# telegraphroad/VCNF

Hardware: AMD Instinct MI355X
Metric: flow transforms/sec (log_prob + sample), D=64 RQ-spline, batch=1M (higher is better)
Workload: dtype f32 results on fp16x3 split operands: every fp32 operand of a conditioner GEMM travels as hi + lo fp16 halves, three f16 matrix instructions per product (four in the 48- and 16-deep layers), fp32 accumulation; measured against fp64 (tests/test_gpu_gemm_error.py): GEMM error 0.6-0.75x the exact-fp32

## Files before the change

### vcnf_amd/csrc/fused_layer_v6.hip

```cpp
#include <hip/hip_runtime.h>
#include <stdint.h>

#include "../../include/vcnf_hip.h"
#include "rqs_math.hpp"
#include "fused_common.hpp"
#include "host_common.hpp"
#include "rqs_lean.hpp"
#include "split_half.hpp"

#ifndef VCNF_ABL
#define VCNF_ABL 0
#endif
#ifndef VCNF_TIME
#define VCNF_TIME 0
#endif
#ifndef VCNF_AHEAD
#define VCNF_AHEAD 1
#endif
#if VCNF_TIME
#define VCNF_T(I) { const long long t_ = clock64(); tacc[I] += t_ - tlast; tlast = t_; }
#define VCNF_TIME_PARAM , float* tstamps
#define VCNF_TIME_ARG , time_buffer()
#else
#define VCNF_T(I)
#define VCNF_TIME_PARAM
#define VCNF_TIME_ARG
#endif

#define VCNF_SYNC() { __builtin_amdgcn_sched_barrier(0); asm volatile("s_waitcnt lgkmcnt(0)\n\ts_barrier" ::: "memory"); __builtin_amdgcn_sched_barrier(0); }

namespace vcnf {

#if VCNF_TIME
constexpr int kTimeSlots = 24;
static float* time_buffer() {
  static float* buf = nullptr;
  if (!buf && hipMalloc(&buf, 2 * kTimeSlots * sizeof(float)) != hipSuccess) buf = nullptr;
  return buf;
}
extern "C" int vcnf_v6_phase_stamps(float* out) {
  if (!time_buffer() || hipDeviceSynchronize() != hipSuccess) return VCNF_ERR_LAUNCH;
  return hipMemcpy(out, time_buffer(), 2 * kTimeSlots * sizeof(float), hipMemcpyDeviceToHost) == hipSuccess ? VCNF_OK : VCNF_ERR_LAUNCH;
}
#endif

template <int DI, int DT, int C, int H, int NBLK, int K, bool INV>
__global__ __launch_bounds__(512, 2) void fused_rqs_layer_v6_kernel(const FusedArgs a VCNF_TIME_PARAM) {
  static_assert(H == 128 && K == 8, "4 row blocks of 32 over 4 waves; 3 K - 1 = 23 logits: two features per 48 rows");
  static_assert((DI == 16 || DI == 32) && DT == DI && (C == 0 || C == 16), "shape family");
  constexpr int kBlock = 512;
  constexpr int kTile = 128;
  constexpr int NCB = 4;
  constexpr int D = DI + DT;
  constexpr int XS = D + 4;
  constexpr int NTX = DI / 16;
  constexpr int NTC = C / 16;
  constexpr int NT0 = NTX + NTC;
  constexpr int NTH = H / 16;
  constexpr int P = 3 * K - 1;
  constexpr int NG = DT / 4;
  constexpr int NR = NG / 2;
  constexpr int TABW = 3 * (K + 1);
  using L = PackLayout6<DI, DT, C, H, NBLK, K>;
  constexpr int GFRAG = 3 * NTH * 2 * 64;
  constexpr int RING = VCNF_AHEAD + 1;

  extern __shared__ __align__(16) float smem[];
  using S = LdsV6<DI, DT, C, H, NBLK, K>;
  static_assert(S::TILE == kTile && S::FRAG_N == 2 * GFRAG * 4 && S::XT_N == kTile * XS && S::TAB_N >= DI * TABW, "layout");
  uint4* act = reinterpret_cast<uint4*>(smem + S::FRAG);
  uint4* act_hi = act;
  uint4* act_lo = act + NTH * NCB * 64;
  float* xt = smem + S::XT;
  uint4* ctxf = reinterpret_cast<uint4*>(smem + S::CTXF);
  float* tab = smem + S::TAB;
  float* ldt = smem + S::LDT;
  int* tfi = reinterpret_cast<int*>(smem + S::TFI);
  int* idi = reinterpret_cast<int*>(smem + S::IDI);
  constexpr int NBV = C > 0 ? 3 : 2;
  constexpr int NBT = S::NBT;
  constexpr int BPL = S::BPL;
  float* biasf = smem + S::BIAS;
  float* ldold = smem + S::LDOLD;
  int* tflag = reinterpret_cast<int*>(smem + S::TFLAG);

  const int tid = threadIdx.x;
  const int lane = tid & 63;
  const int wave = __builtin_amdgcn_readfirstlane(tid >> 6);
  const int rp = wave & 3;
  const int ch = wave >> 2;
  const int c32 = lane & 31;
  const int kg = lane >> 5;
  const RqsConst& c = a.c;
  const bool shared = a.sh_w != nullptr;
  const LeanConst lc = make_lean_const(c);

  if (ch == 1) __builtin_amdgcn_s_setprio(1);
  for (int i = tid; i < NG * 96; i += kBlock) {
    const int g = i / 96, hf = i % 96 / 48;
    biasf[hf * BPL + g * 48 + i % 48] = a.wpack[L::BF + i];
  }
  for (int i = tid; i < NBT * H; i += kBlock) {
    const int v = i / H, blk = (v - 1) / NBV, sel = (v - 1) % NBV, r = i % H;
    const int off = v == 0 ? L::B0 : L::BLK0 + blk * L::BLK + (sel == 0 ? L::BA : sel == 1 ? L::BB : L::BC);
    biasf[(r >> 4 & 1) * BPL + NG * 48 + v * (H / 2) + (r >> 5) * 16 + (r & 15)] = a.wpack[off + r];
  }
  for (int i = tid; i < DT; i += kBlock) tfi[i] = a.tf_idx[i];
  for (int i = tid; i < DI; i += kBlock) idi[i] = a.id_idx[i];
  if (shared) {
    for (int i = tid; i < 3 * DI; i += kBlock) {
      const int f = i % DI;
      SplitLogits p{a.sh_w + f * K, a.sh_h + f * K, a.sh_d + f * (K - 1), K, 1.f, c.edge_logit, c.tails};
      rqs_build_table_part_k<K>(p, c, tab + f * TABW, 1, i / DI);
    }
  }

  const __amdgpu_buffer_rsrc_t wr =
      __builtin_amdgcn_make_buffer_rsrc(const_cast<float*>(a.wpack), 0, a.wpack_bytes, 0x00020000);
  const int voff = lane * 16;
  const float* bplane = biasf + kg * BPL;

  const long long ntiles = (a.B + kTile - 1) / kTile;
  bool bad = false;
  float satm = 0.f;
#if VCNF_TIME
  long long tacc[20], tlast = clock64();
  const long long tstart = tlast, rstart = wall_clock64();
  for (int i = 0; i < 20; ++i) tacc[i] = 0;
#endif
  float4 xpre[kTile * (D / 4) / kBlock], cpre[1];
  static_assert(kTile * (D / 4) % kBlock == 0 && (C == 0 || kTile * (C / 4) == kBlock), "rows per thread");
#define VCNF_PREFETCH_ROWS(TILE)                                                          \
  {                                                                                       \
    const long long pb0 = min((TILE) * kTile, a.B);                                       \
    const long long left = (a.B - pb0) * (D * 4);                                         \
    const __amdgpu_buffer_rsrc_t xr_ = __builtin_amdgcn_make_buffer_rsrc(                 \
        const_cast<float*>(a.x) + pb0 * D, 0, (int)min(left, (long long)(kTile * D * 4)), 0x00020000); \
    _Pragma("unroll") for (int k = 0; k < kTile * (D / 4) / kBlock; ++k)                  \
      xpre[k] = __builtin_bit_cast(float4, __builtin_amdgcn_raw_buffer_load_b128(xr_, (tid + kBlock * k) * 16, 0, 0)); \
    if (C > 0) {                                                                          \
      const long long leftc = (a.B - pb0) * (C * 4);                                      \
      const __amdgpu_buffer_rsrc_t cr_ = __builtin_amdgcn_make_buffer_rsrc(               \
          const_cast<float*>(a.ctx) + pb0 * C, 0, (int)min(leftc, (long long)(kTile * C * 4)), 0x00020000); \
      cpre[0] = __builtin_bit_cast(float4, __builtin_amdgcn_raw_buffer_load_b128(cr_, tid * 16, 0, 0)); \
    }                                                                                     \
  }
#define VCNF_ROWS_ARRIVED()                                                               \
  {                                                                                       \
    _Pragma("unroll") for (int k = 0; k < kTile * (D / 4) / kBlock; ++k) {                \
      floatx4 v_ = __builtin_bit_cast(floatx4, xpre[k]);                                  \
      asm volatile("" : "+v"(v_));                                                        \
      xpre[k] = __builtin_bit_cast(float4, v_);                                           \
    }                                                                                     \
    if (C > 0) {                                                                          \
      floatx4 v_ = __builtin_bit_cast(floatx4, cpre[0]);                                  \
      asm volatile("" : "+v"(v_));                                                        \
      cpre[0] = __builtin_bit_cast(float4, v_);                                           \
    }                                                                                     \
  }
  VCNF_PREFETCH_ROWS((long long)blockIdx.x)
  VCNF_ROWS_ARRIVED()
  for (long long tile = blockIdx.x; tile < ntiles; tile += gridDim.x) {
    const long long b0 = tile * kTile;
    const int rows = (int)min((long long)kTile, a.B - b0);
    satm = 0.f;
    { VCNF_T(0) VCNF_SYNC(); VCNF_T(15) }
    {
      constexpr int D4 = D / 4;
      if (tid == 0) *tflag = 0;
#pragma unroll
      for (int k = 0; k < kTile * D4 / kBlock; ++k) {
        const int i = tid + kBlock * k;
        const int r = i / D4, o = i - r * D4;
        *reinterpret_cast<float4*>(xt + r * XS + 4 * o) = xpre[k];
      }
      if (C > 0) {
        const int r = tid >> 2, part = tid & 3;
        half4 h4, l4;
        const float cv[4] = {cpre[0].x, cpre[0].y, cpre[0].z, cpre[0].w};
#pragma unroll
        for (int i = 0; i < 4; ++i) satm = fmaxf(satm, cv[i] == cv[i] ? __builtin_fabsf(cv[i]) : __builtin_inff());
        asm volatile("" : "+v"(satm));
#pragma unroll
        for (int i = 0; i < 4; ++i) {
          const float x = __builtin_amdgcn_fmed3f(cv[i], -65504.f, 65504.f);
          const _Float16 hv = (_Float16)x;
          h4[i] = hv;
          l4[i] = (_Float16)((x - (float)hv) * kLoScale);
        }
        const int at = (((r >> 5) * 2) * 64 + (r & 31) + 32 * (part >> 1));
        uint2* dh = reinterpret_cast<uint2*>(ctxf + at) + (part & 1);
        uint2* dl = reinterpret_cast<uint2*>(ctxf + at + 64) + (part & 1);
        *dh = __builtin_bit_cast(uint2, h4);
        *dl = __builtin_bit_cast(uint2, l4);
      }
    }
    { VCNF_T(1) VCNF_SYNC(); VCNF_T(15) }

    {
      constexpr int UNR = DI / 4;
      const int mi = tid >> 2, part = tid & 3;
      float lsum = 0.f;
      float xv[UNR], fv[UNR];
      float* px[UNR];
#pragma unroll
      for (int k = 0; k < UNR; ++k) {
        px[k] = xt + mi * XS + idi[part * UNR + k];
        xv[k] = *px[k];
        fv[k] = xv[k];
      }
      if (shared) {
        float yv[UNR], lad[UNR];
        bool in_[UNR];
#pragma unroll
        for (int k = 0; k < UNR; ++k) {
          in_[k] = (xv[k] >= c.lo_x) && (xv[k] <= c.hi_x);
          bool bad1 = false;
          rqs_point_table_inside<INV, K>(in_[k] ? xv[k] : c.lo_x, tab + (part * UNR + k) * TABW, yv[k], lad[k], bad1);
          bad = bad || (bad1 && in_[k]);
        }
#pragma unroll
        for (int k = 0; k < UNR; ++k) {
          const float o = in_[k] ? yv[k] : xv[k];
          *px[k] = o;
          if (INV) fv[k] = o;
          lsum += in_[k] ? lad[k] : 0.f;
        }
      }
      lsum += __shfl_xor(lsum, 1, 64);
      lsum += __shfl_xor(lsum, 2, 64);
      int tid_ = tid;
      asm volatile("" : "+v"(tid_));
      if (part == 0) ldt[tid_ >> 2] = lsum;
#pragma unroll
      for (int k = 0; k < UNR; ++k) satm = fmaxf(satm, fv[k] == fv[k] ? 0.f : __builtin_inff());
      const int k0 = part * UNR;
      const int t0 = k0 >> 4, kg0 = (k0 >> 3) & 1;
      const int at = (t0 * NCB + (mi >> 5)) * 64 + (mi & 31) + 32 * kg0;
      if (UNR == 8) {
        half8 h8, l8;
        float f8[8];
#pragma unroll
        for (int k = 0; k < 8; ++k) f8[k] = fv[k < UNR ? k : 0];
        split8<false>(f8, h8, l8, satm);
        act_hi[at] = __builtin_bit_cast(uint4, h8);
        act_lo[at] = __builtin_bit_cast(uint4, l8);
      } else {
        half4 h4, l4;
        satm = fmaxf(fmaxf(satm, __builtin_fabsf(fv[0])), __builtin_fabsf(fv[1]));
        satm = fmaxf(fmaxf(satm, __builtin_fabsf(fv[2 < UNR ? 2 : 0])), __builtin_fabsf(fv[3 < UNR ? 3 : 0]));
        asm volatile("" : "+v"(satm));
#pragma unroll
        for (int i = 0; i < 4; ++i) {
          const float x = __builtin_amdgcn_fmed3f(fv[i < UNR ? i : 0], -65504.f, 65504.f);
          const _Float16 hv = (_Float16)x;
          h4[i] = hv;
          l4[i] = (_Float16)((x - (float)hv) * kLoScale);
        }
        reinterpret_cast<uint2*>(act_hi + at)[(k0 >> 2) & 1] = __builtin_bit_cast(uint2, h4);
        reinterpret_cast<uint2*>(act_lo + at)[(k0 >> 2) & 1] = __builtin_bit_cast(uint2, l4);
      }
    }
    { VCNF_T(2) VCNF_SYNC(); VCNF_T(15) }
    if (ch == 1) { VCNF_T(14) VCNF_SYNC(); VCNF_T(16) }

    half8 ahi[NTH], alo[NTH];
    floatx16 abias;
#define VCNF_LOAD_BIAS16(DST, VEC)                                                        \
  _Pragma("unroll") for (int i_ = 0; i_ < 4; ++i_) {                                      \
    const floatx4 b4_ = *reinterpret_cast<const floatx4*>(bplane + NG * 48 + (VEC) * (H / 2) + 16 * rp + 4 * i_); \
    DST[4 * i_ + 0] = b4_[0]; DST[4 * i_ + 1] = b4_[1]; DST[4 * i_ + 2] = b4_[2]; DST[4 * i_ + 3] = b4_[3]; \
  }
#define VCNF_LOAD_HIDDEN(WOFF, BVEC)                                                      \
  {                                                                                       \
    _Pragma("unroll") for (int t = 0; t < NTH; ++t) {                                     \
      ahi[t] = __builtin_bit_cast(half8, wload(wr, voff, 4 * ((WOFF) + ((rp * NTH + t) * 2 + 0) * 256))); \
      alo[t] = __builtin_bit_cast(half8, wload(wr, voff, 4 * ((WOFF) + ((rp * NTH + t) * 2 + 1) * 256))); \
    }                                                                                     \
    VCNF_LOAD_BIAS16(abias, BVEC)                                                         \
  }

    floatx16 h[2];
    {
      half8 w0h[NT0], w0l[NT0];
      floatx16 bias0;
#pragma unroll
      for (int t = 0; t < NT0; ++t) {
        w0h[t] = __builtin_bit_cast(half8, wload(wr, voff, 4 * (L::W0 + ((rp * NT0 + t) * 2 + 0) * 256)));
        w0l[t] = __builtin_bit_cast(half8, wload(wr, voff, 4 * (L::W0 + ((rp * NT0 + t) * 2 + 1) * 256)));
      }
      VCNF_LOAD_BIAS16(bias0, 0)
#pragma unroll
      for (int j = 0; j < 2; ++j) {
        const int cb = 2 * ch + j;
        floatx16 mainv = bias0, corr = {}, corr2 = {};
#pragma unroll
        for (int t = 0; t < NT0; ++t) {
          const half8 bh = __builtin_bit_cast(half8, t < NTX ? act_hi[(t * NCB + cb) * 64 + lane] : ctxf[(cb * 2 + 0) * 64 + lane]);
          const half8 bl = __builtin_bit_cast(half8, t < NTX ? act_lo[(t * NCB + cb) * 64 + lane] : ctxf[(cb * 2 + 1) * 64 + lane]);
          mainv = mfma32h(w0h[t], bh, mainv);
          corr = mfma32h(w0h[t], bl, corr);
          corr = mfma32h(w0l[t], bh, corr);
          corr2 = mfma32h(w0l[t], bl, corr2);
        }
#pragma unroll
        for (int r = 0; r < 16; ++r) h[j][r] = fmaf(fmaf(corr2[r], kLoUnscale, corr[r]), kLoUnscale, mainv[r]);
      }
    }
    { VCNF_T(3) VCNF_SYNC(); VCNF_T(15) }
#define VCNF_PUBLISH(SRC, RELU)                                                           \
  _Pragma("unroll") for (int j = 0; j < 2; ++j) {                                         \
    _Pragma("unroll") for (int hh = 0; hh < 2; ++hh) {                                    \
      float v8_[8];                                                                       \
      _Pragma("unroll") for (int i = 0; i < 8; ++i) v8_[i] = SRC[j][8 * hh + i];          \
      half8 h8_, l8_;                                                                     \
      split8<RELU>(v8_, h8_, l8_, satm);                                                  \
      const int at = ((2 * rp + hh) * NCB + 2 * ch + j) * 64 + lane;                      \
      act_hi[at] = __builtin_bit_cast(uint4, h8_);                                        \
      act_lo[at] = __builtin_bit_cast(uint4, l8_);                                        \
    }                                                                                     \
  }
    VCNF_LOAD_HIDDEN(L::BLK0 + L::WA, 1)
    VCNF_PUBLISH(h, true)
    { VCNF_T(4) VCNF_SYNC(); VCNF_T(15) }

#define VCNF_READ_B(T)                                                                    \
  {                                                                                       \
    rh[(T) % RING] = __builtin_bit_cast(half8, act_hi[((((T) & 7)) * NCB + 2 * ch + ((T) >> 3)) * 64 + lane]); \
    rl[(T) % RING] = __builtin_bit_cast(half8, act_lo[((((T) & 7)) * NCB + 2 * ch + ((T) >> 3)) * 64 + lane]); \
  }
#define VCNF_HIDDEN_COMPUTE(OUT)                                                          \
  {                                                                                       \
    half8 rh[RING], rl[RING];                 \
    floatx16 corr;                                                                        \
    _Pragma("unroll") for (int st_ = 0; st_ < VCNF_AHEAD; ++st_) {                        \
      VCNF_READ_B(st_)                                                                    \
    }                                                                                     \
    _Pragma("unroll") for (int st_ = 0; st_ < 2 * NTH; ++st_) {                           \
      const int j = st_ >> 3, tk_ = st_ & 7;                                              \
      if (st_ + VCNF_AHEAD < 2 * NTH) {                                                   \
        VCNF_READ_B(st_ + VCNF_AHEAD)                                                     \
      }                                                                                   \
      if (tk_ == 0) {                                                                       \
        OUT[j] = abias;                                                                   \
        corr = floatx16{};                                                                \
      }                                                                                   \
      OUT[j] = mfma32h(ahi[tk_], rh[st_ % RING], OUT[j]);                                      \
      corr = mfma32h(ahi[tk_], rl[st_ % RING], corr);                                          \
      corr = mfma32h(alo[tk_], rh[st_ % RING], corr);                                          \
      if (tk_ == NTH - 1) {                                                                 \
        _Pragma("unroll") for (int r = 0; r < 16; ++r) OUT[j][r] = fmaf(corr[r], kLoUnscale, OUT[j][r]); \
      }                                                                                   \
    }                                                                                     \
    __builtin_amdgcn_sched_group_barrier(0x100, 2 * VCNF_AHEAD, 0);                       \
    _Pragma("unroll") for (int st_ = 0; st_ + VCNF_AHEAD < 2 * NTH; ++st_) {              \
      __builtin_amdgcn_sched_group_barrier(0x100, 2, 0);                                  \
      __builtin_amdgcn_sched_group_barrier(0x008, 3, 0);                                  \
    }                                                                                     \
    __builtin_amdgcn_sched_group_barrier(0x008, 3 * VCNF_AHEAD, 0);                       \
  }

#pragma unroll
    for (int blk = 0; blk < (VCNF_ABL == 5 ? 0 : NBLK); ++blk) {
      const int base = L::BLK0 + blk * L::BLK;
      floatx16 t[2];
      VCNF_HIDDEN_COMPUTE(t)
      { VCNF_T(5) VCNF_SYNC(); VCNF_T(15) }
      VCNF_LOAD_HIDDEN(base + L::WB, 2 + blk * NBV)
      half8 wch, wcl;
      floatx16 gate[2], gbias;
      if (C > 0) {
        wch = __builtin_bit_cast(half8, wload(wr, voff, 4 * (base + L::WC + (rp * 2 + 0) * 256)));
        wcl = __builtin_bit_cast(half8, wload(wr, voff, 4 * (base + L::WC + (rp * 2 + 1) * 256)));
        VCNF_LOAD_BIAS16(gbias, 3 + blk * NBV)
      }
      VCNF_PUBLISH(t, true)
      { VCNF_T(6) VCNF_SYNC(); VCNF_T(15) }
      VCNF_HIDDEN_COMPUTE(t)
      if (C > 0 && VCNF_ABL != 6) {
#pragma unroll
        for (int j = 0; j < 2; ++j) {
          const half8 bh = __builtin_bit_cast(half8, ctxf[((2 * ch + j) * 2 + 0) * 64 + lane]);
          const half8 bl = __builtin_bit_cast(half8, ctxf[((2 * ch + j) * 2 + 1) * 64 + lane]);
          floatx16 corr = {}, corr2 = {};
          gate[j] = mfma32h(wch, bh, gbias);
          corr = mfma32h(wch, bl, corr);
          corr = mfma32h(wcl, bh, corr);
          corr2 = mfma32h(wcl, bl, corr2);
#pragma unroll
          for (int r = 0; r < 16; ++r) gate[j][r] = fmaf(fmaf(corr2[r], kLoUnscale, corr[r]), kLoUnscale, gate[j][r]);
        }
      }
      { VCNF_T(5) VCNF_SYNC(); VCNF_T(15) }
      if (blk + 1 < NBLK) {
        VCNF_LOAD_HIDDEN(base + L::BLK + L::WA, 1 + (blk + 1) * NBV)
      }
      if (C > 0 && VCNF_ABL != 6) {
#pragma unroll
        for (int j = 0; j < 2; ++j) {
#pragma unroll
          for (int r = 0; r < 16; ++r) {
            const float sg = hw_rcp(1.f + hw_exp2(-gate[j][r]));
            h[j][r] = fmaf(t[j][r], sg, h[j][r]);
          }
        }
      } else {
#pragma unroll
        for (int j = 0; j < 2; ++j) h[j] += t[j];
      }
      if (blk + 1 < NBLK) {
        VCNF_PUBLISH(h, true)
      } else {
        VCNF_PUBLISH(h, false)
      }
      { VCNF_T(7) VCNF_SYNC(); VCNF_T(15) }
    }
    if (ch == 0) { VCNF_T(14) VCNF_SYNC(); VCNF_T(17) }
#undef VCNF_HIDDEN_COMPUTE
#undef VCNF_READ_B
#undef VCNF_LOAD_HIDDEN
#undef VCNF_PUBLISH

    half8 fhi[NTH], flo[NTH];
#pragma unroll
    for (int t = 0; t < NTH; ++t) {
      fhi[t] = __builtin_bit_cast(half8, act_hi[(t * NCB + rp) * 64 + lane]);
      flo[t] = __builtin_bit_cast(half8, act_lo[(t * NCB + rp) * 64 + lane]);
    }
    float ld_acc = 0.f;
    uint4* win = act + ch * GFRAG;
    const int gtid = tid & 255;
    constexpr int NSTG = GFRAG / 256;
    static_assert(GFRAG % 256 == 0, "whole fragments per thread");
#define VCNF_STAGE_DMA(G)                                                                 \
  _Pragma("unroll") for (int k = 0; k < NSTG; ++k)                                        \
    dma16_to_lds(wr, win + (gtid & ~63) + k * 256, gtid * 16, 4 * (L::WF + (G) * (4 * GFRAG) + k * 1024));
    floatx16 pa[3];
#define VCNF_LOAD_BIASF(G)                                                                \
  _Pragma("unroll") for (int b = 0; b < 3; ++b) {                                         \
    _Pragma("unroll") for (int i_ = 0; i_ < 4; ++i_) {                                    \
      const floatx4 b4_ = *reinterpret_cast<const floatx4*>(bplane + (G) * 48 + 16 * b + 4 * i_); \
      pa[b][4 * i_ + 0] = b4_[0]; pa[b][4 * i_ + 1] = b4_[1]; pa[b][4 * i_ + 2] = b4_[2]; pa[b][4 * i_ + 3] = b4_[3]; \
    }                                                                                     \
  }
    VCNF_LOAD_BIASF(ch)
    { VCNF_T(8) VCNF_SYNC(); VCNF_T(15) }
    VCNF_STAGE_DMA(ch)
    if (ch == 0 && rp < 2 && a.ld_mode) {
      const __amdgpu_buffer_rsrc_t or_ = __builtin_amdgcn_make_buffer_rsrc(a.logdet + b0, 0, rows * 4, 0x00020000);
      __builtin_amdgcn_raw_ptr_buffer_load_lds(or_, (__attribute__((address_space(3))) void*)(ldold + rp * 64), 4,
                                               lane * 4, rp * 256, 0, 0);
    }
    wait_vector_memory();
    { VCNF_T(9) VCNF_SYNC(); VCNF_T(15) }
    if (ch == 1) { VCNF_T(14) VCNF_SYNC(); VCNF_T(18) }
    for (int rnd = 0; rnd < (VCNF_ABL == 3 ? 0 : NR); ++rnd) {
      const int g = 2 * rnd + ch;
      float* px[2];
      float xin[2];
#pragma unroll
      for (int f2 = 0; f2 < 2; ++f2) {
        px[f2] = xt + (rp * 32 + c32) * XS + tfi[4 * g + 2 * kg + f2];
        xin[f2] = *px[f2];
      }
      {
        half8 wh[RING], wl[RING];
        floatx16 corr;
#define VCNF_READ_W(T)                                                                    \
  {                                                                                       \
    wh[(T) % RING] = __builtin_bit_cast(half8, win[((T) * 2 + 0) * 64 + lane]);           \
    wl[(T) % RING] = __builtin_bit_cast(half8, win[((T) * 2 + 1) * 64 + lane]);           \
  }
#pragma unroll
        for (int u = 0; u < VCNF_AHEAD; ++u) {
          VCNF_READ_W(u)
        }
#pragma unroll
        for (int u = 0; u < 3 * NTH; ++u) {
          const int b = u >> 3, t = u & 7;
          if (u + VCNF_AHEAD < 3 * NTH) {
            VCNF_READ_W(u + VCNF_AHEAD)
          }
          if (t == 0) corr = floatx16{};
          pa[b] = mfma32h(wh[u % RING], fhi[t], pa[b]);
          corr = mfma32h(wh[u % RING], flo[t], corr);
          corr = mfma32h(wl[u % RING], fhi[t], corr);
          if (t == NTH - 1) {
#pragma unroll
            for (int r = 0; r < 16; ++r) pa[b][r] = fmaf(corr[r], kLoUnscale, pa[b][r]);
          }
        }
        __builtin_amdgcn_sched_group_barrier(0x100, 2 * VCNF_AHEAD, 0);
#pragma unroll
        for (int u = 0; u + VCNF_AHEAD < 3 * NTH; ++u) {
          __builtin_amdgcn_sched_group_barrier(0x100, 2, 0);
          __builtin_amdgcn_sched_group_barrier(0x008, 3, 0);
        }
        __builtin_amdgcn_sched_group_barrier(0x008, 3 * VCNF_AHEAD, 0);
#undef VCNF_READ_W
      }
      { VCNF_T(10) VCNF_SYNC(); VCNF_T(15) }
      {
        const bool more = rnd + 1 < NR;
        if (!more) {
          VCNF_PREFETCH_ROWS(tile + gridDim.x)
        }
        if (more && VCNF_ABL != 2) {
          VCNF_STAGE_DMA(g + 2)
        }
        float yv[2], lad[2];
#pragma unroll
        for (int f2 = 0; f2 < 2; ++f2) {
          float lg[P];
#pragma unroll
          for (int tl = 0; tl < P; ++tl) lg[tl] = pa[(24 * f2 + tl) >> 4][(24 * f2 + tl) & 15];
          rqs_lean_eval<8, INV>(xin[f2], lg, lc, yv[f2], lad[f2], bad);
        }
        *px[0] = yv[0];
        *px[1] = yv[1];
        ld_acc += lad[0] + lad[1];
        if (more) {
          VCNF_LOAD_BIASF(g + 2)
        }
      }
      if (rnd + 1 < NR && VCNF_ABL != 2) wait_vector_memory();
      { VCNF_T(11) VCNF_SYNC(); VCNF_T(15) }
    }
    if (ch == 0) { VCNF_T(14) VCNF_SYNC(); VCNF_T(19) }
#undef VCNF_PREFETCH_ROWS
#undef VCNF_STAGE_DMA
#undef VCNF_LOAD_BIASF

    ld_acc += __shfl_xor(ld_acc, 32, 64);
    if (ch == 1 && kg == 0) ldt[rp * 32 + c32] += ld_acc;
    if (satm > 65504.f) *tflag = 1;
    { VCNF_T(12) VCNF_SYNC(); VCNF_T(15) }
    VCNF_ROWS_ARRIVED()
#undef VCNF_ROWS_ARRIVED
    int tid_ = tid;
    asm volatile("" : "+v"(tid_));
    const bool over = *tflag != 0;
    if (tid == 0 && over && a.sat) atomicAdd(a.sat, 1);
    if (a.redo) {
      if (tid_ < kTile / kFusedFlagRows) {
        const __amdgpu_buffer_rsrc_t rr = __builtin_amdgcn_make_buffer_rsrc(
            a.redo + tile * (kTile / kFusedFlagRows), 0, 4 * ((rows + kFusedFlagRows - 1) / kFusedFlagRows), 0x00020000);
        __builtin_amdgcn_raw_buffer_store_b32(over ? 1 : 0, rr, tid_ * 4, 0, 0);
      }
      if (over) continue;
    }
    if (ch == 0 && (tid_ & 32) == 0) {
      const int mrow = (tid_ >> 6) * 32 + (tid_ & 31);
      const __amdgpu_buffer_rsrc_t lr = __builtin_amdgcn_make_buffer_rsrc(a.logdet + b0, 0, rows * 4, 0x00020000);
      const float o = a.ld_sign * (ld_acc + ldt[mrow]);
      __builtin_amdgcn_raw_buffer_store_b32(__builtin_bit_cast(unsigned, a.ld_mode ? ldold[mrow] + o : o), lr, mrow * 4, 0, 0);
    }
    {
      constexpr int D4 = D / 4;
      const __amdgpu_buffer_rsrc_t yr = __builtin_amdgcn_make_buffer_rsrc(a.y + b0 * D, 0, rows * (D * 4), 0x00020000);
      floatx4 yv[kTile * D4 / kBlock];
#pragma unroll
      for (int k = 0; k < kTile * D4 / kBlock; ++k) {
        const int i = tid_ + kBlock * k;
        const int r = i / D4, o = i - r * D4;
        yv[k] = *reinterpret_cast<const floatx4*>(xt + r * XS + 4 * o);
      }
#pragma unroll
      for (int k = 0; k < kTile * D4 / kBlock; ++k)
        __builtin_amdgcn_raw_buffer_store_b128(__builtin_bit_cast(__attribute__((ext_vector_type(4))) unsigned, yv[k]), yr, (tid_ + kBlock * k) * 16, 0, 0);
    }
  }
#if VCNF_TIME
  VCNF_T(13)
  if (blockIdx.x == 0 && (tid & 255) == 0 && tstamps) {
    float* ts = tstamps + (tid >> 8) * kTimeSlots;
    for (int i = 0; i < 20; ++i) ts[i] = (float)tacc[i];
    ts[20] = (float)(clock64() - tstart);
    ts[21] = (float)(wall_clock64() - rstart);
    ts[22] = (float)((ntiles - blockIdx.x + gridDim.x - 1) / gridDim.x);
  }
#endif
  if (INV && a.bad && bad) atomicAdd(a.bad, 1);
}

template <int DI, int DT, int C, int H, int NBLK, int K>
static int launch_v6(const FusedArgs& a, int inverse, hipStream_t st) {
  constexpr int TILE = 128;
  constexpr size_t lds = LdsV6<DI, DT, C, H, NBLK, K>::BYTES;
  const bool set = inverse ? lds_limit_once<&fused_rqs_layer_v6_kernel<DI, DT, C, H, NBLK, K, true>>(lds)
                           : lds_limit_once<&fused_rqs_layer_v6_kernel<DI, DT, C, H, NBLK, K, false>>(lds);
  if (!set) return VCNF_ERR_LAUNCH;
  const long long ntiles = (a.B + TILE - 1) / TILE;
  dim3 grid((unsigned)(ntiles < 256 ? ntiles : 256));
  if (inverse)
    hipLaunchKernelGGL((fused_rqs_layer_v6_kernel<DI, DT, C, H, NBLK, K, true>), grid, dim3(512), lds, st, a VCNF_TIME_ARG);
  else
    hipLaunchKernelGGL((fused_rqs_layer_v6_kernel<DI, DT, C, H, NBLK, K, false>), grid, dim3(512), lds, st, a VCNF_TIME_ARG);
  return launched();
}

template <int NBLK>
static int launch_v6_family(const FusedArgs& a, int d_id, int ctx_dim, int inverse, hipStream_t st) {
#ifdef VCNF_DEV_ONLY
  return launch_v6<32, 32, 16, 128, NBLK, 8>(a, inverse, st);
#else
  return with_fused_shape(d_id, ctx_dim,
                          [&](auto DI, auto C) { return launch_v6<DI(), DI(), C(), 128, NBLK, 8>(a, inverse, st); });
#endif
}

#ifndef VCNF_V6_NBLK
#define VCNF_V6_NBLK 2
#endif
VCNF_BLOCKS_ENTRY(launch_fused_v6_b, VCNF_V6_NBLK, FusedArgs, launch_v6_family)

}
```

### vcnf_amd/csrc/fused_lds.hpp

```cpp
#pragma once

#include <stddef.h>

namespace vcnf {

template <int DI, int DT, int C, int H, int NBLK, int K>
struct LdsV6 {
  static constexpr int TILE = 128, D = DI + DT, NG = DT / 4;
  static constexpr int NBT = 1 + NBLK * (C > 0 ? 3 : 2);
  static constexpr int BPL = NG * 48 + NBT * (H / 2);
  static constexpr int FRAG = 0, FRAG_N = 2 * 3 * (H / 16) * 2 * 64 * 4;
  static constexpr int XT = FRAG + FRAG_N, XT_N = TILE * (D + 4);
  static constexpr int CTXF = XT + XT_N, CTXF_N = C > 0 ? 4 * 2 * 64 * 4 : 0;
  static constexpr int TAB = CTXF + CTXF_N, TAB_N = (DI * 3 * (K + 1) + 3) & ~3;
  static constexpr int LDT = TAB + TAB_N, LDT_N = TILE;
  static constexpr int TFI = LDT + LDT_N, TFI_N = DT;
  static constexpr int IDI = TFI + TFI_N, IDI_N = DI + 4;
  static constexpr int BIAS = IDI + IDI_N, BIAS_N = 2 * BPL;
  static constexpr int LDOLD = BIAS + BIAS_N, LDOLD_N = TILE;
  static constexpr int TFLAG = LDOLD + LDOLD_N, TFLAG_N = 1;
  static constexpr int END = TFLAG + TFLAG_N;
  static constexpr size_t SLACK_BYTES = 3 * 4 + 64;
  static constexpr size_t BYTES = (size_t)END * 4 + SLACK_BYTES;
  static_assert(FRAG == 0 && FRAG + FRAG_N <= XT && XT + XT_N <= CTXF && CTXF + CTXF_N <= TAB && TAB + TAB_N <= LDT &&
                    LDT + LDT_N <= TFI && TFI + TFI_N <= IDI && IDI + IDI_N <= BIAS && BIAS + BIAS_N <= LDOLD &&
                    LDOLD + LDOLD_N <= TFLAG && (size_t)(TFLAG + TFLAG_N) * 4 <= BYTES,
                "regions in order, none overlaps the next, the last ends within BYTES");
  static_assert(XT % 4 == 0 && CTXF % 4 == 0 && TAB % 4 == 0, "16-byte aligned rows and fragments");
};

template <int DI, int DT, int C, int H, int NBLK, int K>
struct LdsV6s {
  static constexpr int TILE = 32, D = DI + DT, NG = DT / 4;
  static constexpr int TABF = (DI * 3 * (K + 1) + 3) & ~3;
  static constexpr int TSET = TABF + DT + DI + 4 + NG * 96;
  static constexpr int ACT = 0, ACT_N = 4 * (H / 16) * 64 * 4;
  static constexpr int XT = ACT + ACT_N, XT_N = TILE * (D + 4);
  static constexpr int CTXF = XT + XT_N, CTXF_N = C > 0 ? 2 * 64 * 4 : 0;
  static constexpr int LDT = CTXF + CTXF_N, LDT_N = TILE;
  static constexpr int LDX = LDT + LDT_N, LDX_N = 8 * TILE;
  static constexpr int TFLAG = LDX + LDX_N, TFLAG_N = 4;
  static constexpr int TSETS = TFLAG + TFLAG_N, TSETS_N = 2 * TSET;
  static constexpr int END = TSETS + TSETS_N;
  static constexpr size_t SLACK_BYTES = 64;
  static constexpr size_t BYTES = (size_t)END * 4 + SLACK_BYTES;
  static_assert(ACT == 0 && ACT + ACT_N <= XT && XT + XT_N <= CTXF && CTXF + CTXF_N <= LDT && LDT + LDT_N <= LDX &&
                    LDX + LDX_N <= TFLAG && TFLAG + TFLAG_N <= TSETS && (size_t)(TSETS + TSETS_N) * 4 <= BYTES,
                "regions in order, none overlaps the next, the last ends within BYTES");
  static_assert(XT % 4 == 0 && CTXF % 4 == 0 && TSETS % 4 == 0 && TSET % 4 == 0, "16-byte aligned rows and tables");
};

template <int DI, int DT, int C, int H, int NBLK, int K, int kCB>
struct LdsF32 {
  static constexpr int TILE = 4 * kCB * 16, D = DI + DT;
  static constexpr int XT = 0, XT_N = TILE * (D + 4);
  static constexpr int CT = XT + XT_N, CT_N = TILE * ((C > 0 ? C : 4) + 4);
  static constexpr int TAB = CT + CT_N, TAB_N = (DI * 3 * (K + 1) + 3) & ~3;
  static constexpr int TFI = TAB + TAB_N, TFI_N = DT;
  static constexpr int IDI = TFI + TFI_N, IDI_N = DI;
  static constexpr int END = IDI + IDI_N;
  static constexpr size_t SLACK_BYTES = 64;
  static constexpr size_t BYTES = (size_t)END * 4 + SLACK_BYTES;
  static_assert(XT + XT_N <= CT && CT + CT_N <= TAB && TAB + TAB_N <= TFI && TFI + TFI_N <= IDI &&
                    (size_t)(IDI + IDI_N) * 4 <= BYTES,
                "regions in order, none overlaps the next, the last ends within BYTES");
  static_assert(CT % 4 == 0 && TAB % 4 == 0, "16-byte aligned rows");
};

}
```

Baseline: 74.21 million.

## Stage next tile rows via LDS DMA and deepen fragment read-ahead

Next-tile input rows and context are no longer prefetched into registers. They are DMA-loaded straight into LDS stage regions placed inside free parts of the weight/activation fragment window, then copied into the row tile at the start of the tile. This frees the VGPRs that held the row prefetch across the whole round loop. The read-ahead depth for hidden-layer and round fragment reads goes from one to two, except in one shape where it stays at one. The round loop is split so the last round is peeled, and the LDS overlap assumptions are checked with static_asserts.

```diff
diff --git a/vcnf_amd/csrc/fused_layer_v6.hip b/vcnf_amd/csrc/fused_layer_v6.hip
--- a/vcnf_amd/csrc/fused_layer_v6.hip
+++ b/vcnf_amd/csrc/fused_layer_v6.hip
@@ -14,8 +14,11 @@
 #ifndef VCNF_TIME
 #define VCNF_TIME 0
 #endif
-#ifndef VCNF_AHEAD
-#define VCNF_AHEAD 1
+#ifndef VCNF_AHEAD_T
+#define VCNF_AHEAD_T 2
+#endif
+#ifndef VCNF_AHEAD_R
+#define VCNF_AHEAD_R 2
 #endif
 #if VCNF_TIME
 #define VCNF_T(I) { const long long t_ = clock64(); tacc[I] += t_ - tlast; tlast = t_; }
@@ -63,7 +66,8 @@
   constexpr int TABW = 3 * (K + 1);
   using L = PackLayout6<DI, DT, C, H, NBLK, K>;
   constexpr int GFRAG = 3 * NTH * 2 * 64;
-  constexpr int RING = VCNF_AHEAD + 1;
+  constexpr int AHEAD_T = (DI == 32 && C == 16 && NBLK == 3) ? 1 : VCNF_AHEAD_T, AHEAD_R = VCNF_AHEAD_R;
+  constexpr int RING_T = AHEAD_T + 1, RING_R = AHEAD_R + 1;
 
   extern __shared__ __align__(16) float smem[];
   using S = LdsV6<DI, DT, C, H, NBLK, K>;
@@ -128,56 +132,59 @@
   const long long tstart = tlast, rstart = wall_clock64();
   for (int i = 0; i < 20; ++i) tacc[i] = 0;
 #endif
-  float4 xpre[kTile * (D / 4) / kBlock], cpre[1];
-  static_assert(kTile * (D / 4) % kBlock == 0 && (C == 0 || kTile * (C / 4) == kBlock), "rows per thread");
-#define VCNF_PREFETCH_ROWS(TILE)                                                          \
+  constexpr int XS4 = XS / 4;
+  static_assert(S::STG_X_N == 64 * XS4 * 4 && (C == 0 || S::STG_C_N == 4 * 256) && kTile * (D / 4) % (2 * kBlock) == 0, "stage pieces");
+  float* stage = smem + (ch == 0 ? S::STGA : S::STGB);
+#define VCNF_STAGE_ROWS(TILE)                                                             \
   {                                                                                       \
     const long long pb0 = min((TILE) * kTile, a.B);                                       \
     const long long left = (a.B - pb0) * (D * 4);                                         \
     const __amdgpu_buffer_rsrc_t xr_ = __builtin_amdgcn_make_buffer_rsrc(                 \
         const_cast<float*>(a.x) + pb0 * D, 0, (int)min(left, (long long)(kTile * D * 4)), 0x00020000); \
-    _Pragma("unroll") for (int k = 0; k < kTile * (D / 4) / kBlock; ++k)                  \
-      xpre[k] = __builtin_bit_cast(float4, __builtin_amdgcn_raw_buffer_load_b128(xr_, (tid + kBlock * k) * 16, 0, 0)); \
+    _Pragma("unroll") for (int k = 0; k < (XS4 + 3) / 4; ++k) {                           \
+      const int p_ = rp + 4 * k;                                                          \
+      if (p_ < XS4) {                                                                     \
+        const int s_ = p_ * 64 + lane, r_ = s_ / XS4, o_ = s_ - r_ * XS4;                 \
+        dma16_to_lds(xr_, stage + p_ * 256, o_ < D / 4 ? ((ch * 64 + r_) * D + 4 * o_) * 4 : kTile * D * 4, 0); \
+      }                                                                                   \
+    }                                                                                     \
     if (C > 0) {                                                                          \
       const long long leftc = (a.B - pb0) * (C * 4);                                      \
       const __amdgpu_buffer_rsrc_t cr_ = __builtin_amdgcn_make_buffer_rsrc(               \
           const_cast<float*>(a.ctx) + pb0 * C, 0, (int)min(leftc, (long long)(kTile * C * 4)), 0x00020000); \
-      cpre[0] = __builtin_bit_cast(float4, __builtin_amdgcn_raw_buffer_load_b128(cr_, tid * 16, 0, 0)); \
-    }                                                                                     \
-  }
-#define VCNF_ROWS_ARRIVED()                                                               \
-  {                                                                                       \
-    _Pragma("unroll") for (int k = 0; k < kTile * (D / 4) / kBlock; ++k) {                \
-      floatx4 v_ = __builtin_bit_cast(floatx4, xpre[k]);                                  \
-      asm volatile("" : "+v"(v_));                                                        \
-      xpre[k] = __builtin_bit_cast(float4, v_);                                           \
-    }                                                                                     \
-    if (C > 0) {                                                                          \
-      floatx4 v_ = __builtin_bit_cast(floatx4, cpre[0]);                                  \
-      asm volatile("" : "+v"(v_));                                                        \
-      cpre[0] = __builtin_bit_cast(float4, v_);                                           \
-    }                                                                                     \
-  }
-  VCNF_PREFETCH_ROWS((long long)blockIdx.x)
-  VCNF_ROWS_ARRIVED()
+      dma16_to_lds(cr_, stage + S::STG_X_N + rp * 256, tid * 16, 0);                      \
+    }                                                                                     \
+  }
+  VCNF_STAGE_ROWS((long long)blockIdx.x)
+  wait_vector_memory();
   for (long long tile = blockIdx.x; tile < ntiles; tile += gridDim.x) {
     const long long b0 = tile * kTile;
     const int rows = (int)min((long long)kTile, a.B - b0);
     satm = 0.f;
     { VCNF_T(0) VCNF_SYNC(); VCNF_T(15) }
     {
-      constexpr int D4 = D / 4;
+      constexpr int D4 = D / 4, NK = kTile * D4 / kBlock;
       if (tid == 0) *tflag = 0;
-#pragma unroll
-      for (int k = 0; k < kTile * D4 / kBlock; ++k) {
-        const int i = tid + kBlock * k;
+      int tid_ = tid;
+      asm volatile("" : "+v"(tid_));
+      floatx4 xrow[NK];
+#pragma unroll
+      for (int k = 0; k < NK; ++k) {
+        const int i = tid_ + kBlock * k;
         const int r = i / D4, o = i - r * D4;
-        *reinterpret_cast<float4*>(xt + r * XS + 4 * o) = xpre[k];
+        xrow[k] = *reinterpret_cast<const floatx4*>(smem + (k < NK / 2 ? S::STGA : S::STGB) + (r & 63) * XS + 4 * o);
+      }
+#pragma unroll
+      for (int k = 0; k < NK; ++k) {
+        const int i = tid_ + kBlock * k;
+        const int r = i / D4, o = i - r * D4;
+        *reinterpret_cast<floatx4*>(xt + r * XS + 4 * o) = xrow[k];
       }
       if (C > 0) {
-        const int r = tid >> 2, part = tid & 3;
+        const int r = tid_ >> 2, part = tid_ & 3;
         half4 h4, l4;
-        const float cv[4] = {cpre[0].x, cpre[0].y, cpre[0].z, cpre[0].w};
+        const floatx4 cpre = *reinterpret_cast<const floatx4*>(stage + S::STG_X_N + (tid_ & 255) * 4);
+        const float cv[4] = {cpre[0], cpre[1], cpre[2], cpre[3]};
 #pragma unroll
         for (int i = 0; i < 4; ++i) satm = fmaxf(satm, cv[i] == cv[i] ? __builtin_fabsf(cv[i]) : __builtin_inff());
         asm volatile("" : "+v"(satm));
@@ -326,38 +333,38 @@
 
 #define VCNF_READ_B(T)                                                                    \
   {                                                                                       \
-    rh[(T) % RING] = __builtin_bit_cast(half8, act_hi[((((T) & 7)) * NCB + 2 * ch + ((T) >> 3)) * 64 + lane]); \
-    rl[(T) % RING] = __builtin_bit_cast(half8, act_lo[((((T) & 7)) * NCB + 2 * ch + ((T) >> 3)) * 64 + lane]); \
+    rh[(T) % RING_T] = __builtin_bit_cast(half8, act_hi[((((T) & 7)) * NCB + 2 * ch + ((T) >> 3)) * 64 + lane]); \
+    rl[(T) % RING_T] = __builtin_bit_cast(half8, act_lo[((((T) & 7)) * NCB + 2 * ch + ((T) >> 3)) * 64 + lane]); \
   }
 #define VCNF_HIDDEN_COMPUTE(OUT)                                                          \
   {                                                                                       \
-    half8 rh[RING], rl[RING];                 \
+    half8 rh[RING_T], rl[RING_T];             \
     floatx16 corr;                                                                        \
-    _Pragma("unroll") for (int st_ = 0; st_ < VCNF_AHEAD; ++st_) {                        \
+    _Pragma("unroll") for (int st_ = 0; st_ < AHEAD_T; ++st_) {                           \
       VCNF_READ_B(st_)                                                                    \
     }                                                                                     \
     _Pragma("unroll") for (int st_ = 0; st_ < 2 * NTH; ++st_) {                           \
       const int j = st_ >> 3, tk_ = st_ & 7;                                              \
-      if (st_ + VCNF_AHEAD < 2 * NTH) {                                                   \
-        VCNF_READ_B(st_ + VCNF_AHEAD)                                                     \
+      if (st_ + AHEAD_T < 2 * NTH) {                                                      \
+        VCNF_READ_B(st_ + AHEAD_T)                                                        \
       }                                                                                   \
       if (tk_ == 0) {                                                                       \
         OUT[j] = abias;                                                                   \
         corr = floatx16{};                                                                \
       }                                                                                   \
-      OUT[j] = mfma32h(ahi[tk_], rh[st_ % RING], OUT[j]);                                      \
-      corr = mfma32h(ahi[tk_], rl[st_ % RING], corr);                                          \
-      corr = mfma32h(alo[tk_], rh[st_ % RING], corr);                                          \
+      OUT[j] = mfma32h(ahi[tk_], rh[st_ % RING_T], OUT[j]);                               \
+      corr = mfma32h(ahi[tk_], rl[st_ % RING_T], corr);                                   \
+      corr = mfma32h(alo[tk_], rh[st_ % RING_T], corr);                                   \
       if (tk_ == NTH - 1) {                                                                 \
         _Pragma("unroll") for (int r = 0; r < 16; ++r) OUT[j][r] = fmaf(corr[r], kLoUnscale, OUT[j][r]); \
       }                                                                                   \
     }                                                                                     \
-    __builtin_amdgcn_sched_group_barrier(0x100, 2 * VCNF_AHEAD, 0);                       \
-    _Pragma("unroll") for (int st_ = 0; st_ + VCNF_AHEAD < 2 * NTH; ++st_) {              \
+    __builtin_amdgcn_sched_group_barrier(0x100, 2 * AHEAD_T, 0);                          \
+    _Pragma("unroll") for (int st_ = 0; st_ + AHEAD_T < 2 * NTH; ++st_) {                 \
       __builtin_amdgcn_sched_group_barrier(0x100, 2, 0);                                  \
       __builtin_amdgcn_sched_group_barrier(0x008, 3, 0);                                  \
     }                                                                                     \
-    __builtin_amdgcn_sched_group_barrier(0x008, 3 * VCNF_AHEAD, 0);                       \
+    __builtin_amdgcn_sched_group_barrier(0x008, 3 * AHEAD_T, 0);                          \
   }
 
 #pragma unroll
@@ -434,7 +441,7 @@
     static_assert(GFRAG % 256 == 0, "whole fragments per thread");
 #define VCNF_STAGE_DMA(G)                                                                 \
   _Pragma("unroll") for (int k = 0; k < NSTG; ++k)                                        \
-    dma16_to_lds(wr, win + (gtid & ~63) + k * 256, gtid * 16, 4 * (L::WF + (G) * (4 * GFRAG) + k * 1024));
+    dma16_to_lds(wr, win + rp * 64 + k * 256, gtid * 16, 4 * (L::WF + (G) * (4 * GFRAG) + k * 1024));
     floatx16 pa[3];
 #define VCNF_LOAD_BIASF(G)                                                                \
   _Pragma("unroll") for (int b = 0; b < 3; ++b) {                                         \
@@ -448,13 +455,17 @@
     VCNF_STAGE_DMA(ch)
     if (ch == 0 && rp < 2 && a.ld_mode) {
       const __amdgpu_buffer_rsrc_t or_ = __builtin_amdgcn_make_buffer_rsrc(a.logdet + b0, 0, rows * 4, 0x00020000);
+      int lane_ = tid;
+      asm volatile("" : "+v"(lane_));
       __builtin_amdgcn_raw_ptr_buffer_load_lds(or_, (__attribute__((address_space(3))) void*)(ldold + rp * 64), 4,
-                                               lane * 4, rp * 256, 0, 0);
+                                               (lane_ & 63) * 4, rp * 256, 0, 0);
     }
     wait_vector_memory();
     { VCNF_T(9) VCNF_SYNC(); VCNF_T(15) }
     if (ch == 1) { VCNF_T(14) VCNF_SYNC(); VCNF_T(18) }
-    for (int rnd = 0; rnd < (VCNF_ABL == 3 ? 0 : NR); ++rnd) {
+#pragma unroll
+    for (int last = 0; last < 2; ++last)
+    for (int rnd = last ? NR - 1 : 0; rnd < (VCNF_ABL == 3 ? 0 : last ? NR : NR - 1); ++rnd) {
       const int g = 2 * rnd + ch;
       float* px[2];
       float xin[2];
@@ -464,46 +475,46 @@
         xin[f2] = *px[f2];
       }
       {
-        half8 wh[RING], wl[RING];
+        half8 wh[RING_R], wl[RING_R];
         floatx16 corr;
 #define VCNF_READ_W(T)                                                                    \
   {                                                                                       \
-    wh[(T) % RING] = __builtin_bit_cast(half8, win[((T) * 2 + 0) * 64 + lane]);           \
-    wl[(T) % RING] = __builtin_bit_cast(half8, win[((T) * 2 + 1) * 64 + lane]);           \
-  }
-#pragma unroll
-        for (int u = 0; u < VCNF_AHEAD; ++u) {
+    wh[(T) % RING_R] = __builtin_bit_cast(half8, win[((T) * 2 + 0) * 64 + lane]);         \
+    wl[(T) % RING_R] = __builtin_bit_cast(half8, win[((T) * 2 + 1) * 64 + lane]);         \
+  }
+#pragma unroll
+        for (int u = 0; u < AHEAD_R; ++u) {
           VCNF_READ_W(u)
         }
 #pragma unroll
         for (int u = 0; u < 3 * NTH; ++u) {
           const int b = u >> 3, t = u & 7;
-          if (u + VCNF_AHEAD < 3 * NTH) {
-            VCNF_READ_W(u + VCNF_AHEAD)
+          if (u + AHEAD_R < 3 * NTH) {
+            VCNF_READ_W(u + AHEAD_R)
           }
           if (t == 0) corr = floatx16{};
-          pa[b] = mfma32h(wh[u % RING], fhi[t], pa[b]);
-          corr = mfma32h(wh[u % RING], flo[t], corr);
-          corr = mfma32h(wl[u % RING], fhi[t], corr);
+          pa[b] = mfma32h(wh[u % RING_R], fhi[t], pa[b]);
+          corr = mfma32h(wh[u % RING_R], flo[t], corr);
+          corr = mfma32h(wl[u % RING_R], fhi[t], corr);
           if (t == NTH - 1) {
 #pragma unroll
             for (int r = 0; r < 16; ++r) pa[b][r] = fmaf(corr[r], kLoUnscale, pa[b][r]);
           }
         }
-        __builtin_amdgcn_sched_group_barrier(0x100, 2 * VCNF_AHEAD, 0);
-#pragma unroll
-        for (int u = 0; u + VCNF_AHEAD < 3 * NTH; ++u) {
+        __builtin_amdgcn_sched_group_barrier(0x100, 2 * AHEAD_R, 0);
+#pragma unroll
+        for (int u = 0; u + AHEAD_R < 3 * NTH; ++u) {
           __builtin_amdgcn_sched_group_barrier(0x100, 2, 0);
           __builtin_amdgcn_sched_group_barrier(0x008, 3, 0);
         }
-        __builtin_amdgcn_sched_group_barrier(0x008, 3 * VCNF_AHEAD, 0);
+        __builtin_amdgcn_sched_group_barrier(0x008, 3 * AHEAD_R, 0);
 #undef VCNF_READ_W
       }
       { VCNF_T(10) VCNF_SYNC(); VCNF_T(15) }
       {
-        const bool more = rnd + 1 < NR;
+        const bool more = !last;
         if (!more) {
-          VCNF_PREFETCH_ROWS(tile + gridDim.x)
+          VCNF_STAGE_ROWS(tile + gridDim.x)
         }
         if (more && VCNF_ABL != 2) {
           VCNF_STAGE_DMA(g + 2)
@@ -523,11 +534,11 @@
           VCNF_LOAD_BIASF(g + 2)
         }
       }
-      if (rnd + 1 < NR && VCNF_ABL != 2) wait_vector_memory();
+      if (!last && VCNF_ABL != 2) wait_vector_memory();
       { VCNF_T(11) VCNF_SYNC(); VCNF_T(15) }
     }
     if (ch == 0) { VCNF_T(14) VCNF_SYNC(); VCNF_T(19) }
-#undef VCNF_PREFETCH_ROWS
+#undef VCNF_STAGE_ROWS
 #undef VCNF_STAGE_DMA
 #undef VCNF_LOAD_BIASF
 
@@ -535,8 +546,7 @@
     if (ch == 1 && kg == 0) ldt[rp * 32 + c32] += ld_acc;
     if (satm > 65504.f) *tflag = 1;
     { VCNF_T(12) VCNF_SYNC(); VCNF_T(15) }
-    VCNF_ROWS_ARRIVED()
-#undef VCNF_ROWS_ARRIVED
+    wait_vector_memory();
     int tid_ = tid;
     asm volatile("" : "+v"(tid_));
     const bool over = *tflag != 0;
diff --git a/vcnf_amd/csrc/fused_lds.hpp b/vcnf_amd/csrc/fused_lds.hpp
--- a/vcnf_amd/csrc/fused_lds.hpp
+++ b/vcnf_amd/csrc/fused_lds.hpp
@@ -10,6 +10,16 @@
   static constexpr int NBT = 1 + NBLK * (C > 0 ? 3 : 2);
   static constexpr int BPL = NG * 48 + NBT * (H / 2);
   static constexpr int FRAG = 0, FRAG_N = 2 * 3 * (H / 16) * 2 * 64 * 4;
+  static constexpr int ACT_N = 2 * (H / 16) * 4 * 64 * 4;
+  static constexpr int ACT0_N = (DI / 16) * 4 * 64 * 4;
+  static constexpr int STG_ROWS = TILE / 2, STG_X_N = STG_ROWS * (D + 4), STG_C_N = STG_ROWS * C;
+  static constexpr int STG_N = STG_X_N + STG_C_N;
+  static constexpr int STGA = FRAG + ACT0_N, STGB = FRAG + ACT_N;
+  static_assert(STG_X_N % 256 == 0 && STG_C_N % 256 == 0, "whole 1 KiB pieces (one wave instruction each)");
+  static_assert(STGA + STG_N <= FRAG + ACT_N / 2 && STGA + STG_N <= FRAG + FRAG_N / 2,
+                "group A's stage: above the first layer's hi fragments, below the lo fragments, in its window half");
+  static_assert(STGB >= FRAG + FRAG_N / 2 && STGB >= FRAG + ACT_N / 2 + ACT0_N && STGB + STG_N <= FRAG + FRAG_N,
+                "group B's stage: in its window half, above the activation fragments");
   static constexpr int XT = FRAG + FRAG_N, XT_N = TILE * (D + 4);
   static constexpr int CTXF = XT + XT_N, CTXF_N = C > 0 ? 4 * 2 * 64 * 4 : 0;
   static constexpr int TAB = CTXF + CTXF_N, TAB_N = (DI * 3 * (K + 1) + 3) & ~3;
```

Result: no change. 74.70 million (median of 6 runs) (+0.7%).
